# nmndeep/Robust-Segmentation

Hardware: AMD Instinct MI355X
Metric: SEA attack-iterations/sec (UperNet-CNX-T, 512x512) (higher is better)
Workload: dtype f32 (frozen-weight GEMMs on the 16-bit matrix cores by operand splitting: fp16x2 (22 significant bits per operand, 3 MFMA products) forward, fp16x2 (22 significant bits per operand, 3 MFMA products) input gradient; fp32 storage and accumulate)

## Files before the change

devtools/mlp_fused_stamps.py:

```python
#!/usr/bin/env python3
import os
import sys

ROOT = os.path.dirname(os.path.dirname(os.path.abspath(__file__)))
sys.path[:0] = [ROOT, os.path.join(ROOT, "robust-segmentation_amd")]
import torch
from semseg import _native as N

bwd = len(sys.argv) > 1 and sys.argv[1] == "bwd"
C, M = 96, 131072
H = 4 * C
g = torch.Generator(device="cuda").manual_seed(1)
x = torch.randn(M, C, generator=g, device="cuda")
w1 = torch.randn(H, C, generator=g, device="cuda") * 0.05
b1 = torch.randn(H, generator=g, device="cuda") * 0.1
w2 = torch.randn(C, H, generator=g, device="cuda") * 0.03
b2 = torch.randn(C, generator=g, device="cuda") * 0.1
res = torch.randn(M, C, generator=g, device="cuda")
gy = torch.randn(M, C, generator=g, device="cuda") * 1e-3
word = lambda v: torch.tensor([float(v)], dtype=torch.float32, device="cuda").view(torch.int32)
a1, a2 = word(x.abs().max().item() * 1.7), word((x.abs().max() * w1.abs().sum(1) + b1.abs()).max().item())
mul = (w2.abs().sum(0).max() * 1.13).float().reshape(1)
P1, P2 = N.gemm_split_pack(w1, terms=22), N.gemm_split_pack(w2, terms=22)
P2t, P1t = N.gemm_split_pack(w2, trans=True, terms=22), N.gemm_split_pack(w1, trans=True, terms=22)
y = torch.empty(M, C, device="cuda")
WPB = 4
nw = (M + 32 * WPB - 1) // (32 * WPB) * WPB
dbg = torch.zeros(nw, 8, dtype=torch.int64, device="cuda")
p = lambda t: t.data_ptr() if t is not None else None
for _ in range(30):
    N._check(N.lib().sea_mlp_fused_stamps(int(bwd), p(gy), C, p(x), C, p(P1.data), p(b1), p(P2t.data if bwd else P2.data), p(P1t.data),
                                          p(b2), p(res), p(y), M, C, p(a1), p(a2), p(mul), p(dbg), N._stream()), "stamps")
torch.cuda.synchronize()
d = dbg.double().cpu()
names = ["(epilogue, whole kernel: see below)", "interleaved matrix + element-wise work" + (" + first products" if bwd else ""), "wait for the DMA", "barrier"]
tot = d[:, 4].mean().item()
print(f"{'backward' if bwd else 'forward'} C={C} M={M}: {nw} waves, 13 loop iterations, loop total {tot:.0f} ticks per wave (s_memtime = shader cycles)")
for k, n in list(enumerate(names))[1:]:
    print(f"   {n:40s} {d[:, k].mean().item() / 13:8.0f} ticks per iteration   ({100 * d[:, k].mean().item() / tot:4.1f} %)   "
          f"min wave {d[:, k].min().item() / 13:7.0f}  max wave {d[:, k].max().item() / 13:7.0f}")
print(f"   prologue {d[:, 7].mean().item():.0f} ticks per wave (min {d[:, 7].min().item():.0f}, max {d[:, 7].max().item():.0f}); epilogue "
      f"{d[:, 0].mean().item():.0f} (min {d[:, 0].min().item():.0f}, max {d[:, 0].max().item():.0f}); loop {tot:.0f}")
blk = d.view(-1, WPB, 8)
first_round = blk[:256 * 8 // WPB]
print(f"   first 256 blocks: prologue {first_round[:, :, 7].mean().item():.0f}, later blocks: {blk[256 * 8 // WPB:, :, 7].mean().item():.0f}; "
      f"epilogue first {first_round[:, :, 0].mean().item():.0f}, later {blk[256 * 8 // WPB:, :, 0].mean().item():.0f}")
start = d[:, 5]
print(f"   start stamps span {(start.max() - start.min()).item():.0f} ticks over the grid; barrier per wave of a block: "
      + " ".join(f"{blk[:, w, 3].mean().item() / 13:.0f}" for w in range(WPB)))
```

robust-segmentation_amd/csrc/mlp_fused.hip:

```cpp
#include "gemm_split.h"
#include <type_traits>
#include <utility>

namespace sea {

struct MlpArgs {
  const float* x;
  const float* g;
  int64_t ldx, ldg;
  const char* Wa;
  const char* Wu;
  const char* Wb;
  const float* b1;
  const float* b2;
  const float* res;
  int64_t ldres;
  float* y;
  int64_t ldy;
  int M, H, Npad;
  const uint32_t* amax1;
  const uint32_t* amax2;
  unsigned long long* dbg;
  const float* ln_w;
  const float* ln_b;
  float ln_eps;
  const float* amax_mul;
};

__device__ __forceinline__ float erf_small(float x) {
  const float ax = __builtin_fabsf(x);
  const float t = x * x;
  float p = __builtin_fmaf(t, -0x1.268bc2p-11f, 0x1.420828p-8f);
  p = __builtin_fmaf(t, p, -0x1.b5937p-6f);
  p = __builtin_fmaf(t, p, 0x1.ce077cp-4f);
  p = __builtin_fmaf(t, p, -0x1.81266p-2f);
  p = __builtin_fmaf(t, p, 0x1.06eba0p-3f);
  return __builtin_fmaf(ax, p, ax);
}
__device__ __forceinline__ float erf_large_arg(float x) {
  const float ax = __builtin_fabsf(x);
  float q = __builtin_fmaf(ax, 0x1.1d3156p-16f, -0x1.8d129p-12f);
  q = __builtin_fmaf(ax, q, 0x1.f9a6d2p-9f);
  q = __builtin_fmaf(ax, q, -0x1.8c3164p-6f);
  q = __builtin_fmaf(ax, q, 0x1.b4e9c8p-4f);
  q = __builtin_fmaf(ax, q, 0x1.4515fap-1f);
  q = __builtin_fmaf(ax, q, 0x1.078e50p-3f);
  return __builtin_fmaf(ax, q, ax);
}
__device__ __forceinline__ float erf_exp(float q) { return __builtin_expf(-q); }
__device__ __forceinline__ float erf_finish(float x, float small, float ex) {
  return __builtin_copysignf(__builtin_fabsf(x) < 1.0f ? small : 1.0f - ex, x);
}
constexpr float kRsqrt2 = 0.70710678118654752440f;
__device__ __forceinline__ float gelu_finish(float x, float er) { return 0.5f * x * (1.f + er); }
__device__ __forceinline__ float gelu_grad_finish(float x, float er) {
  const float cdf = 0.5f * (1.f + er);
  const float pdf = __expf(-0.5f * x * x) * 0.39894228040143267794f;
  return cdf + x * pdf;
}
__device__ __forceinline__ float erf_nb(float x) { return erf_finish(x, erf_small(x), erf_exp(erf_large_arg(x))); }
__device__ __forceinline__ float gelu_nb(float x) { return gelu_finish(x, erf_nb(x * kRsqrt2)); }
__device__ __forceinline__ float gelu_grad_nb(float x) { return gelu_grad_finish(x, erf_nb(x * kRsqrt2)); }

__global__ __launch_bounds__(256) void gelu_compare_kernel(unsigned long long* out) {
  unsigned long long bad0 = 0, bad1 = 0;
  for (uint64_t i = (uint64_t)blockIdx.x * 256 + threadIdx.x; i < (1ull << 32); i += (uint64_t)gridDim.x * 256) {
    const float x = __uint_as_float((uint32_t)i);
    const float a = gelu_f(x), b = gelu_nb(x), c = gelu_grad_f(x), d = gelu_grad_nb(x);
    bad0 += (__float_as_uint(a) != __float_as_uint(b)) && !(a != a && b != b);
    bad1 += (__float_as_uint(c) != __float_as_uint(d)) && !(c != c && d != d);
  }
  if (bad0) atomicAdd(out, bad0);
  if (bad1) atomicAdd(out + 1, bad1);
}

template <class Fn, int... I>
__device__ __forceinline__ void static_for_impl(Fn&& f, std::integer_sequence<int, I...>) {
  (f(std::integral_constant<int, I>{}), ...);
}
template <int N, class Fn>
__device__ __forceinline__ void static_for(Fn&& f) {
  static_for_impl(f, std::make_integer_sequence<int, N>{});
}


template <int C>
__global__ __launch_bounds__(256) void ln_rows_probe_kernel(const float* x, const float* ln_w, const float* ln_b, float eps, int M,
                                                            float* yn, float* mean, float* rstd) {
  constexpr int KS = C / 16;
  constexpr int LN_KSP = C <= 128 ? 8 : 16;
  const int lane = threadIdx.x & 63, wave = threadIdx.x >> 6;
  const int r = lane & 31, h = lane >> 5;
  int row = (blockIdx.x * 4 + wave) * 32 + r;
  const bool live = row < M;
  row = live ? row : M - 1;
  f32x4 xa[KS][2];
  const float* const xr = x + (int64_t)row * C + 8 * h;
#pragma unroll
  for (int ks = 0; ks < KS; ++ks) {
    xa[ks][0] = *(const f32x4*)(xr + 16 * ks);
    xa[ks][1] = *(const f32x4*)(xr + 16 * ks + 4);
  }
  const float ln_inv_c = 1.f / (float)C;
  auto ln_tree = [&](float (&t)[2][LN_KSP]) __attribute__((always_inline)) -> float {
#pragma unroll
    for (int o = LN_KSP / 2; o > 0; o >>= 1)
#pragma unroll
      for (int i = 0; i < o; ++i) {
        t[0][i] += t[0][i + o];
        t[1][i] += t[1][i + o];
      }
    const float a0 = t[0][0] + __shfl_xor(t[0][0], 32, 64), a1 = t[1][0] + __shfl_xor(t[1][0], 32, 64);
    return a0 + a1;
  };
  float t[2][LN_KSP];
#pragma unroll
  for (int j = 0; j < 2; ++j)
#pragma unroll
    for (int i = 0; i < LN_KSP; ++i) t[j][i] = i < KS ? (xa[i < KS ? i : 0][j][0] + xa[i < KS ? i : 0][j][1]) + (xa[i < KS ? i : 0][j][2] + xa[i < KS ? i : 0][j][3]) : 0.f;
  float mu;
  {
#pragma clang fp contract(off)
    mu = ln_tree(t) * ln_inv_c;
#pragma unroll
    for (int j = 0; j < 2; ++j)
#pragma unroll
      for (int i = 0; i < LN_KSP; ++i) {
        if (i < KS) {
          const float dx = xa[i][j][0] - mu, dy = xa[i][j][1] - mu, dz = xa[i][j][2] - mu, dw = xa[i][j][3] - mu;
          t[j][i] = fmaf(dx, dx, dy * dy) + fmaf(dz, dz, dw * dw);
        } else {
          t[j][i] = 0.f;
        }
      }
  }
  const float rs = rsqrtf(fmaf(ln_tree(t), ln_inv_c, eps));
  if (live) {
#pragma unroll
    for (int ks = 0; ks < KS; ++ks)
#pragma unroll
      for (int j = 0; j < 2; ++j) {
        const f32x4 wv = *(const f32x4*)(ln_w + 16 * ks + 8 * h + 4 * j), bv = *(const f32x4*)(ln_b + 16 * ks + 8 * h + 4 * j);
        f32x4 o;
        {
#pragma clang fp contract(off)
#pragma unroll
          for (int e = 0; e < 4; ++e) o[e] = fmaf((xa[ks][j][e] - mu) * rs, wv[e], bv[e]);
        }
        *(f32x4*)(yn + (int64_t)row * C + 16 * ks + 8 * h + 4 * j) = o;
      }
    if (h == 0) {
      mean[row] = mu;
      rstd[row] = rs;
    }
  }
}

__device__ __forceinline__ f32x16 mfma3(const u32x4 w_hi, const u32x4 w_mid, const u32x4 a_hi, const u32x4 a_mid, f32x16 c) {
  c = __builtin_amdgcn_mfma_f32_32x32x16_f16(__builtin_bit_cast(f16x8, w_hi), __builtin_bit_cast(f16x8, a_mid), c, 0, 0, 0);
  c = __builtin_amdgcn_mfma_f32_32x32x16_f16(__builtin_bit_cast(f16x8, w_mid), __builtin_bit_cast(f16x8, a_hi), c, 0, 0, 0);
  c = __builtin_amdgcn_mfma_f32_32x32x16_f16(__builtin_bit_cast(f16x8, w_hi), __builtin_bit_cast(f16x8, a_hi), c, 0, 0, 0);
  return c;
}

__device__ __forceinline__ void split8(const f32x4 lo, const f32x4 hi4, float sc, u32x4& f_hi, u32x4& f_mid) {
  u32x2 a[2], b[2];
  split4_f16(lo, sc, a);
  split4_f16(hi4, sc, b);
  f_hi = u32x4{a[0][0], a[0][1], b[0][0], b[0][1]};
  f_mid = u32x4{a[1][0], a[1][1], b[1][0], b[1][1]};
}

constexpr int mlp_stage_bytes(int C, bool bwd) { return (bwd ? 3 : 2) * 128 * C; }
constexpr int mlp_cst_bytes(int C, bool bwd) { return (bwd ? 3 : 2) * 4 * C * 4; }
constexpr int mlp_blocks_per_cu(int C, int waves) { return C <= 96 ? 8 / waves : 1; }
constexpr int mlp_lds_bytes(int C, int waves, bool bwd) {
  const int a = 2 * mlp_stage_bytes(C, bwd) + mlp_cst_bytes(C, bwd);
  const int b = waves * 32 * (C + 4) * 4;
  return a > b ? a : b;
}

template <int C, int WAVES, bool BWD, bool PIPE, bool STAMP = false>
__global__ __launch_bounds__(WAVES * 64, (C <= 96 ? 8 : 4) / 4) void mlp_fused_kernel(const MlpArgs p) {
  constexpr int T = WAVES * 64;
  constexpr int KS = C / 16;
  constexpr int NT = C / 32;
  constexpr int ARR = 128 * C;
  constexpr int NARR = BWD ? 3 : 2;
  constexpr int STAGE = NARR * ARR;
  constexpr int PIECES = STAGE / 16;
  constexpr int PER = (PIECES + T - 1) / T;
  static_assert(PIECES % 64 == 0, "whole waves of 16-byte pieces");
  extern __shared__ __attribute__((aligned(16))) char smem[];

  const uint64_t t_entry = STAMP ? __builtin_amdgcn_s_memtime() : 0;
  const int tid = threadIdx.x, lane = tid & 63, wave = tid >> 6;
  const int wave_u = __builtin_amdgcn_readfirstlane(wave);
  const int r = lane & 31, h = lane >> 5;
  const int M = p.M, H = p.H;
  const int NTILE = H / 32;
  const int m0 = ((int)blockIdx.x * WAVES + wave) * 32;
  int row = m0 + r;
  const bool live = row < M;
  row = live ? row : M - 1;

  const uint32_t lane_off = (uint32_t)((lane >> 2) * 64 + (((lane & 3) ^ ((lane >> 4) & 3)) * 16));
  auto dma = [&](char* st, int ja, int jb) __attribute__((always_inline)) {
    ja = ja < NTILE ? ja : NTILE - 1;
    jb = jb < NTILE ? jb : NTILE - 1;
#pragma unroll
    for (int i = 0; i < PER; ++i) {
      const int pcw = wave_u * 64 + T * i;
      if (PIECES % T != 0 && pcw >= PIECES) continue;
      const int arr = pcw / (8 * C), qw = pcw - arr * (8 * C);
      const char* src;
      if (arr < NARR - 1)
        src = (arr == 0 ? p.Wa : p.Wu) + ((int64_t)(qw >> 7) * H + 32 * ja) * 64 + (qw & 127) * 16;
      else {
        const int t = qw / (4 * C);
        src = p.Wb + ((int64_t)(2 * jb + t) * p.Npad) * 64 + (qw - t * (4 * C)) * 16;
      }
      __builtin_amdgcn_global_load_lds((const __attribute__((address_space(1))) void*)(src + lane_off),
                                       (__attribute__((address_space(3))) void*)(st + pcw * 16), 16, 0, 0);
    }
  };
  char* const st0 = smem;
  char* const st1 = smem + STAGE;
  float* const cst = (float*)(smem + 2 * STAGE);
  {
    const float* const wa_g = (const float*)(p.Wa + (int64_t)(C / 32) * 2 * H * 64);
    const float* const wu_g = BWD ? (const float*)(p.Wu + (int64_t)(C / 32) * 2 * H * 64) : nullptr;
    for (int i = tid; i < H; i += T) {
      cst[i] = wa_g[i];
      cst[H + i] = p.b1[i];
      if constexpr (BWD) cst[2 * H + i] = wu_g[i];
    }
  }
  dma(st1, 0, 0);
  dma(st0, 1, 0);

  constexpr int LDP = (C + 4) * 4;
  constexpr int NF4 = 32 * C / 4 / 64;
  auto load_rows = [&](const float* base, int64_t ld, f32x4 (&out)[KS][2]) __attribute__((always_inline)) {
    const float* const xr = base + (int64_t)row * ld + 8 * h;
#pragma unroll
    for (int ks = 0; ks < KS; ++ks) {
      out[ks][0] = *(const f32x4*)(xr + 16 * ks);
      out[ks][1] = *(const f32x4*)(xr + 16 * ks + 4);
    }
  };
  float sc1, inv1;
  pow2_scale(*p.amax1, sc1, inv1);
  u32x4 xf[KS][2];
  constexpr int LN_KSP = C <= 128 ? 8 : 16;
  const float ln_inv_c = 1.f / (float)C;
  auto ln_tree = [&](float (&t)[2][LN_KSP]) __attribute__((always_inline)) -> float {
#pragma unroll
    for (int o = LN_KSP / 2; o > 0; o >>= 1)
#pragma unroll
      for (int i = 0; i < o; ++i) {
        t[0][i] += t[0][i + o];
        t[1][i] += t[1][i + o];
      }
    const float a0 = t[0][0] + __shfl_xor(t[0][0], 32, 64), a1 = t[1][0] + __shfl_xor(t[1][0], 32, 64);
    return a0 + a1;
  };
  float ln_mu = 0.f, ln_rs = 1.f;
  {
    f32x4 xa[KS][2];
    load_rows(p.x, p.ldx, xa);
    if (p.ln_w != nullptr) {
      float t[2][LN_KSP];
#pragma unroll
      for (int j = 0; j < 2; ++j)
#pragma unroll
        for (int i = 0; i < LN_KSP; ++i) t[j][i] = i < KS ? (xa[i < KS ? i : 0][j][0] + xa[i < KS ? i : 0][j][1]) + (xa[i < KS ? i : 0][j][2] + xa[i < KS ? i : 0][j][3]) : 0.f;
      {
#pragma clang fp contract(off)
        ln_mu = ln_tree(t) * ln_inv_c;
#pragma unroll
        for (int j = 0; j < 2; ++j)
#pragma unroll
          for (int i = 0; i < LN_KSP; ++i) {
            if (i < KS) {
              const float dx = xa[i][j][0] - ln_mu, dy = xa[i][j][1] - ln_mu, dz = xa[i][j][2] - ln_mu, dw = xa[i][j][3] - ln_mu;
              t[j][i] = fmaf(dx, dx, dy * dy) + fmaf(dz, dz, dw * dw);
            } else {
              t[j][i] = 0.f;
            }
          }
      }
      ln_rs = rsqrtf(fmaf(ln_tree(t), ln_inv_c, p.ln_eps));
#pragma unroll
      for (int ks = 0; ks < KS; ++ks)
#pragma unroll
        for (int j = 0; j < 2; ++j) {
          const f32x4 wv = *(const f32x4*)(p.ln_w + 16 * ks + 8 * h + 4 * j), bv = *(const f32x4*)(p.ln_b + 16 * ks + 8 * h + 4 * j);
          {
#pragma clang fp contract(off)
#pragma unroll
            for (int e = 0; e < 4; ++e) xa[ks][j][e] = fmaf((xa[ks][j][e] - ln_mu) * ln_rs, wv[e], bv[e]);
          }
        }
    }
#pragma unroll
    for (int ks = 0; ks < KS; ++ks) split8(xa[ks][0], xa[ks][1], sc1, xf[ks][0], xf[ks][1]);
  }
  float sc2 = 1.f, inv2 = 1.f;
  float invg = 1.f;
  u32x4 gf[BWD ? KS : 1][2];
  if constexpr (BWD) {
    f32x4 ga[KS][2];
    load_rows(p.g, p.ldg, ga);
    uint32_t mx = 0;
#pragma unroll
    for (int ks = 0; ks < KS; ++ks) {
#pragma unroll
      for (int e = 0; e < 4; ++e) {
        const uint32_t b0 = __float_as_uint(ga[ks][0][e]) & 0x7fffffffu, b1 = __float_as_uint(ga[ks][1][e]) & 0x7fffffffu;
        mx = b0 > mx ? b0 : mx;
        mx = b1 > mx ? b1 : mx;
      }
    }
    const uint32_t other = (uint32_t)__shfl_xor((int)mx, 32, 64);
    mx = other > mx ? other : mx;
    float scg;
    pow2_scale(mx, scg, invg);
    const float mul = *p.amax_mul;
    uint32_t word = mx;
    if (mul != 1.f) word = __float_as_uint(__uint_as_float(word) * mul) & 0x7fffffffu;
    pow2_scale(word, sc2, inv2);
#pragma unroll
    for (int ks = 0; ks < KS; ++ks) split8(ga[ks][0], ga[ks][1], scg, gf[ks][0], gf[ks][1]);
  } else {
    pow2_scale(*p.amax2, sc2, inv2);
  }

  asm volatile("s_waitcnt vmcnt(0)" ::: "memory");
  __syncthreads();

  const uint32_t rd = (uint32_t)(r * 64 + swz<false>(r, h));
  auto first = [&](const char* st, f32x16& Tt, f32x16& Ut) __attribute__((always_inline)) {
#pragma unroll
    for (int e = 0; e < 16; ++e) Tt[e] = 0.f;
    if constexpr (BWD) {
#pragma unroll
      for (int e = 0; e < 16; ++e) Ut[e] = 0.f;
    }
#pragma unroll
    for (int ks = 0; ks < KS; ++ks) {
      const uint32_t o = (uint32_t)((ks >> 1) * 4096) + (rd ^ (uint32_t)(32 * (ks & 1)));
      const u32x4 w0 = *(const u32x4*)(st + o), w1 = *(const u32x4*)(st + o + 2048);
      Tt = mfma3(w0, w1, xf[ks][0], xf[ks][1], Tt);
      if constexpr (BWD) {
        const u32x4 u0 = *(const u32x4*)(st + ARR + o), u1 = *(const u32x4*)(st + ARR + o + 2048);
        Ut = mfma3(u0, u1, gf[ks][0], gf[ks][1], Ut);
      }
    }
  };

  f32x16 acc[NT];
#pragma unroll
  for (int n = 0; n < NT; ++n)
#pragma unroll
    for (int e = 0; e < 16; ++e) acc[n][e] = 0.f;

  f32x16 Tc, Uc, Tn, Un;
  first(st1, Tc, Uc);
  __syncthreads();

  const float* const wi_a = cst;
  const float* const b1_l = cst + H;
  const float* const wi_u = cst + 2 * H;
  constexpr int SECOND = (NARR - 1) * ARR;

  u32x4 hp[2][2] = {};
  uint64_t tick[4] = {0, 0, 0, 0};
  const uint64_t t_begin = STAMP ? __builtin_amdgcn_s_memtime() : 0;
#define SEA_PIN() __builtin_amdgcn_sched_barrier(0)
  auto body = [&](auto FF, auto SS, auto EE, int j) __attribute__((always_inline)) {
    constexpr bool F = decltype(FF)::value, S = decltype(SS)::value, E = decltype(EE)::value;
    char* const cur = (j & 1) ? st1 : st0;
    char* const nxt = (j & 1) ? st0 : st1;
    uint64_t c0 = 0, c2 = 0, c3 = 0, c4 = 0;
    if constexpr (STAMP) {
      c0 = __builtin_amdgcn_s_memtime();
      SEA_PIN();
    }
    constexpr bool LAG = PIPE;
    if (j + 1 < NTILE + (LAG ? 1 : 0)) dma(nxt, j + 2, LAG ? j : j + 1);
    constexpr int NTF = (F && PIPE) ? (BWD ? 2 : 1) * KS : 0;
    constexpr int NTS = (S && LAG) ? 2 * NT : 0;
    constexpr int NTR = NTF + NTS, NM = 3 * NTR;
    u32x4 wf[2][2];
    auto rd_frags = [&](auto TR) __attribute__((always_inline)) {
      constexpr int tr = decltype(TR)::value;
      if constexpr (tr < NTF) {
        constexpr int ks = BWD ? tr >> 1 : tr;
        const uint32_t o = (uint32_t)(((BWD && (tr & 1)) ? ARR : 0) + (ks >> 1) * 4096) + (rd ^ (uint32_t)(32 * (ks & 1)));
        wf[tr & 1][0] = *(const u32x4*)(cur + o);
        wf[tr & 1][1] = *(const u32x4*)(cur + o + 2048);
      } else {
        constexpr int t2 = tr - NTF, ss = t2 / NT, n = t2 - ss * NT;
        const uint32_t o = (uint32_t)(SECOND + n * 2048) + (rd ^ (uint32_t)(32 * ss));
        wf[tr & 1][0] = *(const u32x4*)(cur + o);
        wf[tr & 1][1] = *(const u32x4*)(cur + o + C * 64);
      }
    };
    auto mfma_m = [&](auto MC) __attribute__((always_inline)) {
      constexpr int m = decltype(MC)::value, tr = m / 3, pr = m - 3 * tr;
      if constexpr (pr == 0 && tr + 1 < NTR) rd_frags(std::integral_constant<int, tr + 1>{});
      const f16x8 w = __builtin_bit_cast(f16x8, wf[tr & 1][pr == 1 ? 1 : 0]);
      constexpr int at = pr == 0 ? 1 : 0;
      if constexpr (tr < NTF) {
        constexpr int ks = BWD ? tr >> 1 : tr;
        if constexpr (BWD && (tr & 1)) {
          if constexpr (tr == 1 && pr == 0) {
#pragma unroll
            for (int e = 0; e < 16; ++e) Un[e] = 0.f;
          }
          Un = __builtin_amdgcn_mfma_f32_32x32x16_f16(w, __builtin_bit_cast(f16x8, gf[BWD ? ks : 0][at]), Un, 0, 0, 0);
        } else {
          if constexpr (tr == 0 && pr == 0) {
#pragma unroll
            for (int e = 0; e < 16; ++e) Tn[e] = 0.f;
          }
          Tn = __builtin_amdgcn_mfma_f32_32x32x16_f16(w, __builtin_bit_cast(f16x8, xf[ks][at]), Tn, 0, 0, 0);
        }
      } else {
        constexpr int t2 = tr - NTF, ss = t2 / NT, n = t2 - ss * NT;
        acc[n] = __builtin_amdgcn_mfma_f32_32x32x16_f16(w, __builtin_bit_cast(f16x8, hp[ss][at]), acc[n], 0, 0, 0);
      }
    };
    if constexpr (NTR > 0) rd_frags(std::integral_constant<int, 0>{});
    u32x4 hf[2][2];
    if constexpr (E) {
      constexpr int EPS = 4;
      constexpr int SPQ = 2 + 4 * (4 / EPS);
      constexpr int NSTEP = 4 * SPQ + 1;
      float ev[16], ek[16], ep[16], eq[16];
      uint32_t hq[4][2], mq[4][2];
      f32x4 wa, bb, wu;
      auto cst_rd = [&](int q) __attribute__((always_inline)) {
        const int hid = 32 * j + 8 * q + 4 * h;
        wa = *(const f32x4*)(wi_a + hid);
        bb = *(const f32x4*)(b1_l + hid);
        if constexpr (BWD) wu = *(const f32x4*)(wi_u + hid);
      };
      cst_rd(0);
      static_for<NSTEP>([&](auto IC) __attribute__((always_inline)) {
        constexpr int i = decltype(IC)::value;
        constexpr int m0 = i * NM / NSTEP, m1 = (i + 1) * NM / NSTEP;
        static_for<m1 - m0>([&](auto U) __attribute__((always_inline)) { mfma_m(std::integral_constant<int, m0 + decltype(U)::value>{}); });
        constexpr int q = i / SPQ, k = i - SPQ * q;
        if constexpr (i == NSTEP - 1) {
#pragma unroll
          for (int s2 = 0; s2 < 2; ++s2) {
            const auto a0 = __builtin_amdgcn_permlane32_swap(hq[2 * s2][0], hq[2 * s2 + 1][0], false, false);
            const auto a1 = __builtin_amdgcn_permlane32_swap(hq[2 * s2][1], hq[2 * s2 + 1][1], false, false);
            const auto b0 = __builtin_amdgcn_permlane32_swap(mq[2 * s2][0], mq[2 * s2 + 1][0], false, false);
            const auto b1 = __builtin_amdgcn_permlane32_swap(mq[2 * s2][1], mq[2 * s2 + 1][1], false, false);
            hf[s2][0] = u32x4{a0[0], a1[0], a0[1], a1[1]};
            hf[s2][1] = u32x4{b0[0], b1[0], b0[1], b1[1]};
          }
        } else if constexpr (k == 0) {
#pragma unroll
          for (int e = 0; e < 4; ++e) {
            const float t = Tc[4 * q + e] * (inv1 * wa[e]) + bb[e];
            ev[4 * q + e] = t;
            ek[4 * q + e] = t * kRsqrt2;
          }
        } else if constexpr (k == SPQ - 1) {
          u32x2 s2[2];
          split4_f16(f32x4{ev[4 * q], ev[4 * q + 1], ev[4 * q + 2], ev[4 * q + 3]}, sc2, s2);
          hq[q][0] = s2[0][0];
          hq[q][1] = s2[0][1];
          mq[q][0] = s2[1][0];
          mq[q][1] = s2[1][1];
          if constexpr (q + 1 < 4) cst_rd(q + 1);
        } else {
          constexpr int pr = (k - 1) >> 2, st = (k - 1) & 3;
#pragma unroll
          for (int d = 0; d < EPS; ++d) {
            const int e = 4 * q + EPS * pr + d;
            if constexpr (st == 0) ep[e] = erf_small(ek[e]);
            if constexpr (st == 1) eq[e] = erf_large_arg(ek[e]);
            if constexpr (st == 2) eq[e] = erf_exp(eq[e]);
            if constexpr (st == 3) {
              const float er = erf_finish(ek[e], ep[e], eq[e]);
              if constexpr (BWD) {
                float u = Uc[e] * (invg * wu[e & 3]) + 0.f;
                u *= gelu_grad_finish(ev[e], er);
                ev[e] = u;
              } else {
                ev[e] = gelu_finish(ev[e], er);
              }
            }
          }
        }
        SEA_PIN();
      });
    } else {
      static_for<NM>([&](auto MC) __attribute__((always_inline)) { mfma_m(MC); });
    }
    if constexpr (S && !LAG) {
#pragma unroll
      for (int ss = 0; ss < 2; ++ss)
#pragma unroll
        for (int n = 0; n < NT; ++n) {
          const uint32_t o = (uint32_t)(SECOND + n * 2048) + (rd ^ (uint32_t)(32 * ss));
          const u32x4 w0 = *(const u32x4*)(cur + o), w1 = *(const u32x4*)(cur + o + C * 64);
          acc[n] = mfma3(w0, w1, hf[ss][0], hf[ss][1], acc[n]);
        }
    }
    if constexpr (F && !PIPE) first(cur, Tc, Uc);
    if constexpr (E && LAG) {
#pragma unroll
      for (int s2 = 0; s2 < 2; ++s2) {
        hp[s2][0] = hf[s2][0];
        hp[s2][1] = hf[s2][1];
      }
    }
    if constexpr (STAMP) {
      SEA_PIN();
      c2 = __builtin_amdgcn_s_memtime();
      SEA_PIN();
    }
    asm volatile("s_waitcnt vmcnt(0)" ::: "memory");
    if constexpr (STAMP) {
      c3 = __builtin_amdgcn_s_memtime();
      SEA_PIN();
    }
    __syncthreads();
    if constexpr (STAMP) {
      c4 = __builtin_amdgcn_s_memtime();
      SEA_PIN();
      tick[0] += 0;
      tick[1] += c2 - c0;
      tick[2] += c3 - c2;
      tick[3] += c4 - c3;
    }
    if constexpr (F && PIPE) {
      Tc = Tn;
      if constexpr (BWD) Uc = Un;
    }
  };
#undef SEA_PIN
  using Y = std::true_type;
  using No = std::false_type;
  if constexpr (PIPE) {
    body(Y{}, No{}, Y{}, 0);
    for (int j = 1; j + 1 < NTILE; ++j) body(Y{}, Y{}, Y{}, j);
    body(No{}, Y{}, Y{}, NTILE - 1);
    body(No{}, Y{}, No{}, NTILE);
  } else {
    for (int j = 0; j + 1 < NTILE; ++j) body(Y{}, Y{}, Y{}, j);
    body(No{}, Y{}, Y{}, NTILE - 1);
  }
  const uint64_t t_loop_end = STAMP ? __builtin_amdgcn_s_memtime() : 0;

  const float* const wi_b = (const float*)(p.Wb + (int64_t)(H / 32) * 2 * p.Npad * 64);
  {
    char* const ep = smem + wave_u * (32 * LDP);
#pragma unroll
    for (int n = 0; n < NT; ++n)
#pragma unroll
      for (int q = 0; q < 4; ++q) {
        const int col = 32 * n + 8 * q + 4 * h;
        const f32x4 wb = *(const f32x4*)(wi_b + col);
        f32x4 bb = {0.f, 0.f, 0.f, 0.f};
        if (!BWD && p.b2) bb = *(const f32x4*)(p.b2 + col);
        f32x4 v;
#pragma unroll
        for (int e = 0; e < 4; ++e) v[e] = acc[n][4 * q + e] * (inv2 * wb[e]) + bb[e];
        if constexpr (BWD) {
          if (p.ln_w != nullptr) {
#pragma unroll
            for (int e = 0; e < 4; ++e) acc[n][4 * q + e] = v[e];
            continue;
          }
        }
        *(f32x4*)(ep + r * LDP + col * 4) = v;
      }
    if constexpr (BWD) {
      if (p.ln_w != nullptr) {
        constexpr int NTP = C <= 128 ? 4 : 8;
        const float* const xr = p.x + (int64_t)row * p.ldx;
        float t1[NTP][4], t2[NTP][4];
        f32x4 gw[NT][4], xh[NT][4];
#pragma unroll
        for (int n = 0; n < NTP; ++n)
#pragma unroll
          for (int q = 0; q < 4; ++q) {
            if (n < NT) {
              const int col = 32 * n + 8 * q + 4 * h;
              const f32x4 wv = *(const f32x4*)(p.ln_w + col), xv = *(const f32x4*)(xr + col);
              const int nn = n < NT ? n : 0;
              {
#pragma clang fp contract(off)
#pragma unroll
                for (int e = 0; e < 4; ++e) {
                  gw[nn][q][e] = acc[nn][4 * q + e] * wv[e];
                  xh[nn][q][e] = (xv[e] - ln_mu) * ln_rs;
                }
                t1[n][q] = (gw[nn][q][0] + gw[nn][q][1]) + (gw[nn][q][2] + gw[nn][q][3]);
                t2[n][q] = (gw[nn][q][0] * xh[nn][q][0] + gw[nn][q][1] * xh[nn][q][1]) + (gw[nn][q][2] * xh[nn][q][2] + gw[nn][q][3] * xh[nn][q][3]);
              }
            } else {
              t1[n][q] = 0.f;
              t2[n][q] = 0.f;
            }
          }
#pragma unroll
        for (int o = NTP / 2; o > 0; o >>= 1)
#pragma unroll
          for (int i = 0; i < o; ++i)
#pragma unroll
            for (int q = 0; q < 4; ++q) {
              t1[i][q] += t1[i + o][q];
              t2[i][q] += t2[i + o][q];
            }
        float s1 = (t1[0][0] + t1[0][2]) + (t1[0][1] + t1[0][3]), s2 = (t2[0][0] + t2[0][2]) + (t2[0][1] + t2[0][3]);
        s1 += __shfl_xor(s1, 32, 64);
        s2 += __shfl_xor(s2, 32, 64);
#pragma unroll
        for (int n = 0; n < NT; ++n)
#pragma unroll
          for (int q = 0; q < 4; ++q) {
            f32x4 o4;
            {
#pragma clang fp contract(off)
              const float m1 = s1 * ln_inv_c, m2 = s2 * ln_inv_c;
#pragma unroll
              for (int e = 0; e < 4; ++e) o4[e] = ln_rs * fmaf(-xh[n][q][e], m2, gw[n][q][e] - m1);
            }
            *(f32x4*)(ep + r * LDP + (32 * n + 8 * q + 4 * h) * 4) = o4;
          }
      }
    }
    const bool has_res = !BWD && p.res != nullptr;
#pragma unroll
    for (int it = 0; it < NF4; ++it) {
      const int f = lane + 64 * it, rw = f / (C / 4), c4 = f - rw * (C / 4);
      f32x4 v = *(const f32x4*)(ep + rw * LDP + c4 * 16);
      if (m0 + rw < M) {
        if (has_res) v += *(const f32x4*)(p.res + (int64_t)(m0 + rw) * p.ldres + 4 * c4);
        *(f32x4*)(p.y + (int64_t)(m0 + rw) * p.ldy + 4 * c4) = v;
      }
    }
  }
  if constexpr (STAMP) {
    asm volatile("s_waitcnt vmcnt(0)" ::: "memory");
    if (lane == 0 && p.dbg) {
      unsigned long long* d = p.dbg + ((int64_t)blockIdx.x * WAVES + wave) * 8;
      for (int k = 1; k < 4; ++k) d[k] = tick[k];
      d[0] = __builtin_amdgcn_s_memtime() - t_loop_end;
      d[4] = t_loop_end - t_begin;
      d[5] = t_begin;
      d[6] = __builtin_amdgcn_s_memrealtime();
      d[7] = t_begin - t_entry;
    }
  }
}

template <int C, int WAVES, bool BWD, bool PIPE, bool STAMP = false>
static int mlp_launch(const MlpArgs& p, hipStream_t st) {
  constexpr int lds = mlp_lds_bytes(C, WAVES, BWD);
  static_assert(lds * mlp_blocks_per_cu(C, WAVES) <= 160 * 1024, "LDS of a compute unit");
  auto k = mlp_fused_kernel<C, WAVES, BWD, PIPE, STAMP>;
  if (lds > 48 * 1024) {
    static bool attr_set_dev[64] = {};
    int dev = 0;
    (void)hipGetDevice(&dev);
    if (!attr_set_dev[dev & 63]) {
      (void)hipFuncSetAttribute((const void*)k, hipFuncAttributeMaxDynamicSharedMemorySize, lds);
      attr_set_dev[dev & 63] = true;
    }
  }
  const int rows_per_block = WAVES * 32;
  hipLaunchKernelGGL(k, dim3((p.M + rows_per_block - 1) / rows_per_block), dim3(WAVES * 64), (size_t)lds, st, p);
  return (int)hipGetLastError();
}

}

using namespace sea;

extern "C" int sea_probe_gelu_mismatches(unsigned long long* out, void* stream) {
  SEA_CHECK_ARG(out != nullptr);
  hipLaunchKernelGGL(gelu_compare_kernel, dim3(256 * 16), dim3(256), 0, (hipStream_t)stream, out);
  SEA_RETURN_LAST();
}

extern "C" int sea_probe_ln_rows(const float* x, const float* ln_w, const float* ln_b, float eps, int M, int C, float* yn, float* mean,
                                 float* rstd, void* stream) {
  SEA_CHECK_ARG(x && ln_w && ln_b && yn && mean && rstd && M > 0 && (C == 96 || C == 192));
  const dim3 grid((M + 127) / 128), block(256);
  if (C == 96)
    hipLaunchKernelGGL(ln_rows_probe_kernel<96>, grid, block, 0, (hipStream_t)stream, x, ln_w, ln_b, eps, M, yn, mean, rstd);
  else
    hipLaunchKernelGGL(ln_rows_probe_kernel<192>, grid, block, 0, (hipStream_t)stream, x, ln_w, ln_b, eps, M, yn, mean, rstd);
  SEA_RETURN_LAST();
}

extern "C" int sea_mlp_fused_supported(int C, int H) { return (H == 4 * C && (C == 96 || C == 192)) ? 1 : 0; }

static bool mlp_common_ok(const MlpArgs& p, int C) {
  return p.x && p.Wa && p.Wb && p.b1 && p.y && p.amax1 && p.M > 0 && sea_mlp_fused_supported(C, p.H) && (p.ldx % 4) == 0 &&
         (p.ldy % 4) == 0 && p.ldx >= C && p.ldy >= C &&
         ((((uintptr_t)p.x) | ((uintptr_t)p.y) | ((uintptr_t)p.Wa) | ((uintptr_t)p.Wb) | ((uintptr_t)p.b1)) & 15) == 0;
}

static int mlp_fwd_impl(const float* x, int64_t ldx, const void* W1p, const float* b1, const void* W2p, const float* b2,
                        const float* res, int64_t ldres, float* y, int64_t ldy, int M, int C, int H, const uint32_t* amax_x,
                        const uint32_t* amax_h, const float* ln_w, const float* ln_b, float ln_eps, void* stream) {
  MlpArgs p = {};
  p.ln_w = ln_w; p.ln_b = ln_b; p.ln_eps = ln_eps;
  SEA_CHECK_ARG((ln_w == nullptr) == (ln_b == nullptr) && ((((uintptr_t)ln_w) | ((uintptr_t)ln_b)) & 15) == 0);
  p.x = x; p.ldx = ldx; p.Wa = (const char*)W1p; p.Wb = (const char*)W2p; p.b1 = b1; p.b2 = b2; p.res = res; p.ldres = ldres;
  p.y = y; p.ldy = ldy; p.M = M; p.H = H; p.Npad = (C + GS_BN - 1) / GS_BN * GS_BN; p.amax1 = amax_x; p.amax2 = amax_h;
  SEA_CHECK_ARG(mlp_common_ok(p, C) && amax_h != nullptr);
  SEA_CHECK_ARG((((uintptr_t)b2) & 15) == 0 && (!res || ((ldres % 4) == 0 && ldres >= C && (((uintptr_t)res) & 15) == 0)));
  const hipStream_t st = (hipStream_t)stream;
  if (C == 96) return mlp_launch<96, 4, false, true>(p, st);
  return mlp_launch<192, 4, false, true>(p, st);
}

extern "C" int sea_mlp_fused_fwd(const float* x, int64_t ldx, const void* W1p, const float* b1, const void* W2p, const float* b2,
                                 const float* res, int64_t ldres, float* y, int64_t ldy, int M, int C, int H,
                                 const uint32_t* amax_x, const uint32_t* amax_h, void* stream) {
  return mlp_fwd_impl(x, ldx, W1p, b1, W2p, b2, res, ldres, y, ldy, M, C, H, amax_x, amax_h, nullptr, nullptr, 0.f, stream);
}
extern "C" int sea_ln_mlp_fused_fwd(const float* x, int64_t ldx, const float* ln_w, const float* ln_b, float ln_eps, const void* W1p,
                                    const float* b1, const void* W2p, const float* b2, const float* res, int64_t ldres, float* y,
                                    int64_t ldy, int M, int C, int H, const uint32_t* amax_x, const uint32_t* amax_h, void* stream) {
  SEA_CHECK_ARG(ln_w && ln_b);
  return mlp_fwd_impl(x, ldx, W1p, b1, W2p, b2, res, ldres, y, ldy, M, C, H, amax_x, amax_h, ln_w, ln_b, ln_eps, stream);
}

static int mlp_bwd_impl(const float* g, int64_t ldg, const float* x, int64_t ldx, const void* W1p, const float* b1,
                        const void* W2tp, const void* W1tp, float* dx, int64_t lddx, int M, int C, int H, const uint32_t* amax_x,
                        const float* amax_mul_dev, const float* ln_w, const float* ln_b, float ln_eps, void* stream) {
  MlpArgs p = {};
  p.ln_w = ln_w; p.ln_b = ln_b; p.ln_eps = ln_eps;
  SEA_CHECK_ARG((ln_w == nullptr) == (ln_b == nullptr) && ((((uintptr_t)ln_w) | ((uintptr_t)ln_b)) & 15) == 0);
  p.x = x; p.ldx = ldx; p.g = g; p.ldg = ldg; p.Wa = (const char*)W1p; p.Wu = (const char*)W2tp; p.Wb = (const char*)W1tp;
  p.b1 = b1; p.y = dx; p.ldy = lddx; p.M = M; p.H = H; p.Npad = (C + GS_BN - 1) / GS_BN * GS_BN; p.amax1 = amax_x;
  p.amax_mul = amax_mul_dev;
  SEA_CHECK_ARG(mlp_common_ok(p, C) && g && W2tp && amax_mul_dev && (ldg % 4) == 0 && ldg >= C &&
                ((((uintptr_t)g) | ((uintptr_t)W2tp)) & 15) == 0);
  const hipStream_t st = (hipStream_t)stream;
  if (C == 96) return mlp_launch<96, 4, true, false>(p, st);
  return mlp_launch<192, 4, true, true>(p, st);
}

extern "C" int sea_mlp_fused_bwd(const float* g, int64_t ldg, const float* x, int64_t ldx, const void* W1p, const float* b1,
                                 const void* W2tp, const void* W1tp, float* dx, int64_t lddx, int M, int C, int H,
                                 const uint32_t* amax_x, const float* amax_mul_dev, void* stream) {
  return mlp_bwd_impl(g, ldg, x, ldx, W1p, b1, W2tp, W1tp, dx, lddx, M, C, H, amax_x, amax_mul_dev, nullptr, nullptr, 0.f, stream);
}
extern "C" int sea_ln_mlp_fused_bwd(const float* g, int64_t ldg, const float* x, int64_t ldx, const float* ln_w, const float* ln_b,
                                    float ln_eps, const void* W1p, const float* b1, const void* W2tp, const void* W1tp, float* dx,
                                    int64_t lddx, int M, int C, int H, const uint32_t* amax_x, const float* amax_mul_dev,
                                    void* stream) {
  SEA_CHECK_ARG(ln_w && ln_b);
  return mlp_bwd_impl(g, ldg, x, ldx, W1p, b1, W2tp, W1tp, dx, lddx, M, C, H, amax_x, amax_mul_dev, ln_w, ln_b, ln_eps, stream);
}

extern "C" int sea_mlp_fused_stamps(int bwd, const float* g, int64_t ldg, const float* x, int64_t ldx, const void* W1p, const float* b1,
                                    const void* W2p, const void* W1tp, const float* b2, const float* res, float* y, int M, int C,
                                    const uint32_t* amax_x, const uint32_t* amax_h, const float* amax_mul_dev,
                                    unsigned long long* dbg, void* stream) {
  SEA_CHECK_ARG(C == 96 && dbg && x && y);
  MlpArgs p = {};
  p.x = x; p.ldx = ldx; p.g = g; p.ldg = ldg; p.Wa = (const char*)W1p; p.b1 = b1; p.y = y; p.ldy = C; p.M = M; p.H = 4 * C;
  p.Npad = (C + GS_BN - 1) / GS_BN * GS_BN; p.amax1 = amax_x; p.amax2 = amax_h; p.amax_mul = amax_mul_dev; p.dbg = dbg;
  if (bwd) {
    p.Wu = (const char*)W2p; p.Wb = (const char*)W1tp;
    return mlp_launch<96, 4, true, false, true>(p, (hipStream_t)stream);
  }
  p.Wb = (const char*)W2p; p.b2 = b2; p.res = res; p.ldres = C;
  return mlp_launch<96, 4, false, true, true>(p, (hipStream_t)stream);
}
```

Measured before the change: 571.3.

## Split C=192 fused MLP forward across wave pairs with LDS exchange

For the C=192 forward MLP, each 32-row group is now handled by two waves (8 waves per block). One wave runs the first GEMM and half the GELU/split epilogue, the other does the remaining epilogue quarters and the second GEMM. They exchange hidden fragments and T values through a double-buffered LDS slot. This aims to raise occupancy and overlap matrix and element-wise work at the C=192 stage, at the cost of extra LDS, barriers and a role imbalance between the two waves.

```diff
diff --git a/devtools/mlp_fused_stamps.py b/devtools/mlp_fused_stamps.py
--- a/devtools/mlp_fused_stamps.py
+++ b/devtools/mlp_fused_stamps.py
@@ -8,7 +8,8 @@
 from semseg import _native as N
 
 bwd = len(sys.argv) > 1 and sys.argv[1] == "bwd"
-C, M = 96, 131072
+C = int(sys.argv[2]) if len(sys.argv) > 2 else 96
+M = 131072 if C == 96 else 32768
 H = 4 * C
 g = torch.Generator(device="cuda").manual_seed(1)
 x = torch.randn(M, C, generator=g, device="cuda")
@@ -24,8 +25,10 @@
 P1, P2 = N.gemm_split_pack(w1, terms=22), N.gemm_split_pack(w2, terms=22)
 P2t, P1t = N.gemm_split_pack(w2, trans=True, terms=22), N.gemm_split_pack(w1, trans=True, terms=22)
 y = torch.empty(M, C, device="cuda")
-WPB = 4
-nw = (M + 32 * WPB - 1) // (32 * WPB) * WPB
+WPB = int(sys.argv[3]) if len(sys.argv) > 3 else (8 if C == 192 and not bwd else 4)
+RPB = 128
+nw = (M + RPB - 1) // RPB * WPB
+NIT = H // 32 + 1
 dbg = torch.zeros(nw, 8, dtype=torch.int64, device="cuda")
 p = lambda t: t.data_ptr() if t is not None else None
 for _ in range(30):
@@ -35,10 +38,10 @@
 d = dbg.double().cpu()
 names = ["(epilogue, whole kernel: see below)", "interleaved matrix + element-wise work" + (" + first products" if bwd else ""), "wait for the DMA", "barrier"]
 tot = d[:, 4].mean().item()
-print(f"{'backward' if bwd else 'forward'} C={C} M={M}: {nw} waves, 13 loop iterations, loop total {tot:.0f} ticks per wave (s_memtime = shader cycles)")
+print(f"{'backward' if bwd else 'forward'} C={C} M={M}: {nw} waves, {NIT} loop iterations, loop total {tot:.0f} ticks per wave (s_memtime = shader cycles)")
 for k, n in list(enumerate(names))[1:]:
-    print(f"   {n:40s} {d[:, k].mean().item() / 13:8.0f} ticks per iteration   ({100 * d[:, k].mean().item() / tot:4.1f} %)   "
-          f"min wave {d[:, k].min().item() / 13:7.0f}  max wave {d[:, k].max().item() / 13:7.0f}")
+    print(f"   {n:40s} {d[:, k].mean().item() / NIT:8.0f} ticks per iteration   ({100 * d[:, k].mean().item() / tot:4.1f} %)   "
+          f"min wave {d[:, k].min().item() / NIT:7.0f}  max wave {d[:, k].max().item() / NIT:7.0f}")
 print(f"   prologue {d[:, 7].mean().item():.0f} ticks per wave (min {d[:, 7].min().item():.0f}, max {d[:, 7].max().item():.0f}); epilogue "
       f"{d[:, 0].mean().item():.0f} (min {d[:, 0].min().item():.0f}, max {d[:, 0].max().item():.0f}); loop {tot:.0f}")
 blk = d.view(-1, WPB, 8)
@@ -47,4 +50,7 @@
       f"epilogue first {first_round[:, :, 0].mean().item():.0f}, later {blk[256 * 8 // WPB:, :, 0].mean().item():.0f}")
 start = d[:, 5]
 print(f"   start stamps span {(start.max() - start.min()).item():.0f} ticks over the grid; barrier per wave of a block: "
-      + " ".join(f"{blk[:, w, 3].mean().item() / 13:.0f}" for w in range(WPB)))
+      + " ".join(f"{blk[:, w, 3].mean().item() / NIT:.0f}" for w in range(WPB)))
+print("   per wave of a block, work ticks per iteration: " + " ".join(f"{blk[:, w, 1].mean().item() / NIT:.0f}" for w in range(WPB))
+      + "; prologue: " + " ".join(f"{blk[:, w, 7].mean().item():.0f}" for w in range(WPB))
+      + "; epilogue: " + " ".join(f"{blk[:, w, 0].mean().item():.0f}" for w in range(WPB)))
diff --git a/robust-segmentation_amd/csrc/mlp_fused.hip b/robust-segmentation_amd/csrc/mlp_fused.hip
--- a/robust-segmentation_amd/csrc/mlp_fused.hip
+++ b/robust-segmentation_amd/csrc/mlp_fused.hip
@@ -173,16 +173,22 @@
 
 constexpr int mlp_stage_bytes(int C, bool bwd) { return (bwd ? 3 : 2) * 128 * C; }
 constexpr int mlp_cst_bytes(int C, bool bwd) { return (bwd ? 3 : 2) * 4 * C * 4; }
+constexpr bool mlp_paired(int C, bool bwd) { return C == 192 && !bwd; }
+constexpr int mlp_groups(int C, int waves, bool bwd) { return mlp_paired(C, bwd) ? waves / 2 : waves; }
+constexpr int mlp_xchg_bytes(int C, int waves, bool bwd) { return mlp_paired(C, bwd) ? (waves / 2) * 2 * 4096 : 0; }
 constexpr int mlp_blocks_per_cu(int C, int waves) { return C <= 96 ? 8 / waves : 1; }
 constexpr int mlp_lds_bytes(int C, int waves, bool bwd) {
-  const int a = 2 * mlp_stage_bytes(C, bwd) + mlp_cst_bytes(C, bwd);
-  const int b = waves * 32 * (C + 4) * 4;
+  const int a = 2 * mlp_stage_bytes(C, bwd) + mlp_cst_bytes(C, bwd) + mlp_xchg_bytes(C, waves, bwd);
+  const int b = mlp_groups(C, waves, bwd) * 32 * (C + 4) * 4;
   return a > b ? a : b;
 }
 
 template <int C, int WAVES, bool BWD, bool PIPE, bool STAMP = false>
-__global__ __launch_bounds__(WAVES * 64, (C <= 96 ? 8 : 4) / 4) void mlp_fused_kernel(const MlpArgs p) {
+__global__ __launch_bounds__(WAVES * 64, (C <= 96 || mlp_paired(C, BWD)) ? 2 : 1) void mlp_fused_kernel(const MlpArgs p) {
   constexpr int T = WAVES * 64;
+  constexpr bool PAIR = mlp_paired(C, BWD);
+  constexpr int GROUPS = mlp_groups(C, WAVES, BWD);
+  static_assert(!PAIR || (PIPE && WAVES == 8), "the paired form is the pipelined loop at two waves per SIMD");
   constexpr int KS = C / 16;
   constexpr int NT = C / 32;
   constexpr int ARR = 128 * C;
@@ -199,7 +205,8 @@
   const int r = lane & 31, h = lane >> 5;
   const int M = p.M, H = p.H;
   const int NTILE = H / 32;
-  const int m0 = ((int)blockIdx.x * WAVES + wave) * 32;
+  const int grp = PAIR ? wave_u % GROUPS : wave_u, role = PAIR ? wave_u / GROUPS : 0;
+  const int m0 = ((int)blockIdx.x * GROUPS + grp) * 32;
   int row = m0 + r;
   const bool live = row < M;
   row = live ? row : M - 1;
@@ -227,6 +234,7 @@
   char* const st0 = smem;
   char* const st1 = smem + STAGE;
   float* const cst = (float*)(smem + 2 * STAGE);
+  char* const xch = smem + 2 * STAGE + mlp_cst_bytes(C, BWD) + grp * 8192 + lane * 16;
   {
     const float* const wa_g = (const float*)(p.Wa + (int64_t)(C / 32) * 2 * H * 64);
     const float* const wu_g = BWD ? (const float*)(p.Wu + (int64_t)(C / 32) * 2 * H * 64) : nullptr;
@@ -266,7 +274,7 @@
     return a0 + a1;
   };
   float ln_mu = 0.f, ln_rs = 1.f;
-  {
+  auto load_x = [&]() __attribute__((always_inline)) {
     f32x4 xa[KS][2];
     load_rows(p.x, p.ldx, xa);
     if (p.ln_w != nullptr) {
@@ -305,7 +313,8 @@
     }
 #pragma unroll
     for (int ks = 0; ks < KS; ++ks) split8(xa[ks][0], xa[ks][1], sc1, xf[ks][0], xf[ks][1]);
-  }
+  };
+  if constexpr (!PAIR) load_x();
   float sc2 = 1.f, inv2 = 1.f;
   float invg = 1.f;
   u32x4 gf[BWD ? KS : 1][2];
@@ -336,8 +345,11 @@
     pow2_scale(*p.amax2, sc2, inv2);
   }
 
-  asm volatile("s_waitcnt vmcnt(0)" ::: "memory");
-  __syncthreads();
+  auto landed = [&]() __attribute__((always_inline)) {
+    asm volatile("s_waitcnt vmcnt(0)" ::: "memory");
+    __syncthreads();
+  };
+  if constexpr (!PAIR) landed();
 
   const uint32_t rd = (uint32_t)(r * 64 + swz<false>(r, h));
   auto first = [&](const char* st, f32x16& Tt, f32x16& Ut) __attribute__((always_inline)) {
@@ -366,8 +378,10 @@
     for (int e = 0; e < 16; ++e) acc[n][e] = 0.f;
 
   f32x16 Tc, Uc, Tn, Un;
-  first(st1, Tc, Uc);
-  __syncthreads();
+  if constexpr (!PAIR) {
+    first(st1, Tc, Uc);
+    __syncthreads();
+  }
 
   const float* const wi_a = cst;
   const float* const b1_l = cst + H;
@@ -376,10 +390,11 @@
 
   u32x4 hp[2][2] = {};
   uint64_t tick[4] = {0, 0, 0, 0};
-  const uint64_t t_begin = STAMP ? __builtin_amdgcn_s_memtime() : 0;
+  uint64_t t_begin = (STAMP && !PAIR) ? __builtin_amdgcn_s_memtime() : 0;
 #define SEA_PIN() __builtin_amdgcn_sched_barrier(0)
-  auto body = [&](auto FF, auto SS, auto EE, int j) __attribute__((always_inline)) {
+  auto body = [&](auto FF, auto SS, auto EE, auto RRC, int j) __attribute__((always_inline)) {
     constexpr bool F = decltype(FF)::value, S = decltype(SS)::value, E = decltype(EE)::value;
+    constexpr int RR = decltype(RRC)::value;
     char* const cur = (j & 1) ? st1 : st0;
     char* const nxt = (j & 1) ? st0 : st1;
     uint64_t c0 = 0, c2 = 0, c3 = 0, c4 = 0;
@@ -434,10 +449,23 @@
     };
     if constexpr (NTR > 0) rd_frags(std::integral_constant<int, 0>{});
     u32x4 hf[2][2];
+    f32x4 te[2];
+    if constexpr (RR == 2) {
+      const char* const sl = xch + ((j + 1) & 1) * 4096;
+      if constexpr (S) {
+        hp[0][0] = *(const u32x4*)(sl);
+        hp[0][1] = *(const u32x4*)(sl + 1024);
+      }
+      if constexpr (E) {
+        te[0] = *(const f32x4*)(sl + 2048);
+        te[1] = *(const f32x4*)(sl + 3072);
+      }
+    }
     if constexpr (E) {
       constexpr int EPS = 4;
       constexpr int SPQ = 2 + 4 * (4 / EPS);
-      constexpr int NSTEP = 4 * SPQ + 1;
+      constexpr int NQ = RR ? 2 : 4, QB = RR == 2 ? 2 : 0;
+      constexpr int NSTEP = NQ * SPQ + 1;
       float ev[16], ek[16], ep[16], eq[16];
       uint32_t hq[4][2], mq[4][2];
       f32x4 wa, bb, wu;
@@ -447,7 +475,7 @@
         bb = *(const f32x4*)(b1_l + hid);
         if constexpr (BWD) wu = *(const f32x4*)(wi_u + hid);
       };
-      cst_rd(0);
+      cst_rd(QB);
       static_for<NSTEP>([&](auto IC) __attribute__((always_inline)) {
         constexpr int i = decltype(IC)::value;
         constexpr int m0 = i * NM / NSTEP, m1 = (i + 1) * NM / NSTEP;
@@ -455,18 +483,21 @@
         constexpr int q = i / SPQ, k = i - SPQ * q;
         if constexpr (i == NSTEP - 1) {
 #pragma unroll
-          for (int s2 = 0; s2 < 2; ++s2) {
+          for (int s2 = 0; s2 < NQ / 2; ++s2) {
             const auto a0 = __builtin_amdgcn_permlane32_swap(hq[2 * s2][0], hq[2 * s2 + 1][0], false, false);
             const auto a1 = __builtin_amdgcn_permlane32_swap(hq[2 * s2][1], hq[2 * s2 + 1][1], false, false);
             const auto b0 = __builtin_amdgcn_permlane32_swap(mq[2 * s2][0], mq[2 * s2 + 1][0], false, false);
             const auto b1 = __builtin_amdgcn_permlane32_swap(mq[2 * s2][1], mq[2 * s2 + 1][1], false, false);
-            hf[s2][0] = u32x4{a0[0], a1[0], a0[1], a1[1]};
-            hf[s2][1] = u32x4{b0[0], b1[0], b0[1], b1[1]};
+            hf[QB / 2 + s2][0] = u32x4{a0[0], a1[0], a0[1], a1[1]};
+            hf[QB / 2 + s2][1] = u32x4{b0[0], b1[0], b0[1], b1[1]};
           }
         } else if constexpr (k == 0) {
 #pragma unroll
           for (int e = 0; e < 4; ++e) {
-            const float t = Tc[4 * q + e] * (inv1 * wa[e]) + bb[e];
+            float tq;
+            if constexpr (RR == 2) tq = te[q][e];
+            else tq = Tc[4 * q + e];
+            const float t = tq * (inv1 * wa[e]) + bb[e];
             ev[4 * q + e] = t;
             ek[4 * q + e] = t * kRsqrt2;
           }
@@ -477,7 +508,7 @@
           hq[q][1] = s2[0][1];
           mq[q][0] = s2[1][0];
           mq[q][1] = s2[1][1];
-          if constexpr (q + 1 < 4) cst_rd(q + 1);
+          if constexpr (q + 1 < NQ) cst_rd(QB + q + 1);
         } else {
           constexpr int pr = (k - 1) >> 2, st = (k - 1) & 3;
 #pragma unroll
@@ -514,11 +545,22 @@
         }
     }
     if constexpr (F && !PIPE) first(cur, Tc, Uc);
-    if constexpr (E && LAG) {
-#pragma unroll
-      for (int s2 = 0; s2 < 2; ++s2) {
+    if constexpr (E && LAG && RR != 1) {
+#pragma unroll
+      for (int s2 = RR ? 1 : 0; s2 < 2; ++s2) {
         hp[s2][0] = hf[s2][0];
         hp[s2][1] = hf[s2][1];
+      }
+    }
+    if constexpr (RR == 1) {
+      char* const sl = xch + (j & 1) * 4096;
+      if constexpr (E) {
+        *(u32x4*)(sl) = hf[0][0];
+        *(u32x4*)(sl + 1024) = hf[0][1];
+      }
+      if constexpr (F) {
+        *(f32x4*)(sl + 2048) = f32x4{Tn[8], Tn[9], Tn[10], Tn[11]};
+        *(f32x4*)(sl + 3072) = f32x4{Tn[12], Tn[13], Tn[14], Tn[15]};
       }
     }
     if constexpr (STAMP) {
@@ -546,22 +588,9 @@
     }
   };
 #undef SEA_PIN
-  using Y = std::true_type;
-  using No = std::false_type;
-  if constexpr (PIPE) {
-    body(Y{}, No{}, Y{}, 0);
-    for (int j = 1; j + 1 < NTILE; ++j) body(Y{}, Y{}, Y{}, j);
-    body(No{}, Y{}, Y{}, NTILE - 1);
-    body(No{}, Y{}, No{}, NTILE);
-  } else {
-    for (int j = 0; j + 1 < NTILE; ++j) body(Y{}, Y{}, Y{}, j);
-    body(No{}, Y{}, Y{}, NTILE - 1);
-  }
-  const uint64_t t_loop_end = STAMP ? __builtin_amdgcn_s_memtime() : 0;
-
   const float* const wi_b = (const float*)(p.Wb + (int64_t)(H / 32) * 2 * p.Npad * 64);
-  {
-    char* const ep = smem + wave_u * (32 * LDP);
+  char* const ep = smem + grp * (32 * LDP);
+  auto to_patch = [&]() __attribute__((always_inline)) {
 #pragma unroll
     for (int n = 0; n < NT; ++n)
 #pragma unroll
@@ -582,6 +611,46 @@
         }
         *(f32x4*)(ep + r * LDP + col * 4) = v;
       }
+  };
+  uint64_t t_loop_end = 0;
+  using Y = std::true_type;
+  using No = std::false_type;
+  using R0 = std::integral_constant<int, 0>;
+  if constexpr (PAIR) {
+    if (role == 0) {
+      load_x();
+      landed();
+      first(st1, Tc, Uc);
+      *(f32x4*)(xch + 4096 + 2048) = f32x4{Tc[8], Tc[9], Tc[10], Tc[11]};
+      *(f32x4*)(xch + 4096 + 3072) = f32x4{Tc[12], Tc[13], Tc[14], Tc[15]};
+      __syncthreads();
+      if constexpr (STAMP) t_begin = __builtin_amdgcn_s_memtime();
+      for (int j = 0; j + 1 < NTILE; ++j) body(Y{}, No{}, Y{}, std::integral_constant<int, 1>{}, j);
+      body(No{}, No{}, Y{}, std::integral_constant<int, 1>{}, NTILE - 1);
+      body(No{}, No{}, No{}, std::integral_constant<int, 1>{}, NTILE);
+    } else {
+      landed();
+      __syncthreads();
+      if constexpr (STAMP) t_begin = __builtin_amdgcn_s_memtime();
+      body(No{}, No{}, Y{}, std::integral_constant<int, 2>{}, 0);
+      for (int j = 1; j < NTILE; ++j) body(No{}, Y{}, Y{}, std::integral_constant<int, 2>{}, j);
+      body(No{}, Y{}, No{}, std::integral_constant<int, 2>{}, NTILE);
+      if constexpr (STAMP) t_loop_end = __builtin_amdgcn_s_memtime();
+      to_patch();
+    }
+  } else if constexpr (PIPE) {
+    body(Y{}, No{}, Y{}, R0{}, 0);
+    for (int j = 1; j + 1 < NTILE; ++j) body(Y{}, Y{}, Y{}, R0{}, j);
+    body(No{}, Y{}, Y{}, R0{}, NTILE - 1);
+    body(No{}, Y{}, No{}, R0{}, NTILE);
+  } else {
+    for (int j = 0; j + 1 < NTILE; ++j) body(Y{}, Y{}, Y{}, R0{}, j);
+    body(No{}, Y{}, Y{}, R0{}, NTILE - 1);
+  }
+  if (STAMP && !(PAIR && role == 1)) t_loop_end = __builtin_amdgcn_s_memtime();
+
+  {
+    if constexpr (!PAIR) to_patch();
     if constexpr (BWD) {
       if (p.ln_w != nullptr) {
         constexpr int NTP = C <= 128 ? 4 : 8;
@@ -639,8 +708,11 @@
       }
     }
     const bool has_res = !BWD && p.res != nullptr;
-#pragma unroll
-    for (int it = 0; it < NF4; ++it) {
+    if constexpr (PAIR) __syncthreads();
+    constexpr int NIT = PAIR ? NF4 / 2 : NF4;
+#pragma unroll
+    for (int i = 0; i < NIT; ++i) {
+      const int it = PAIR ? role * NIT + i : i;
       const int f = lane + 64 * it, rw = f / (C / 4), c4 = f - rw * (C / 4);
       f32x4 v = *(const f32x4*)(ep + rw * LDP + c4 * 16);
       if (m0 + rw < M) {
@@ -677,7 +749,7 @@
       attr_set_dev[dev & 63] = true;
     }
   }
-  const int rows_per_block = WAVES * 32;
+  const int rows_per_block = mlp_groups(C, WAVES, BWD) * 32;
   hipLaunchKernelGGL(k, dim3((p.M + rows_per_block - 1) / rows_per_block), dim3(WAVES * 64), (size_t)lds, st, p);
   return (int)hipGetLastError();
 }
@@ -723,7 +795,7 @@
   SEA_CHECK_ARG((((uintptr_t)b2) & 15) == 0 && (!res || ((ldres % 4) == 0 && ldres >= C && (((uintptr_t)res) & 15) == 0)));
   const hipStream_t st = (hipStream_t)stream;
   if (C == 96) return mlp_launch<96, 4, false, true>(p, st);
-  return mlp_launch<192, 4, false, true>(p, st);
+  return mlp_launch<192, 8, false, true>(p, st);
 }
 
 extern "C" int sea_mlp_fused_fwd(const float* x, int64_t ldx, const void* W1p, const float* b1, const void* W2p, const float* b2,
@@ -771,14 +843,16 @@
                                     const void* W2p, const void* W1tp, const float* b2, const float* res, float* y, int M, int C,
                                     const uint32_t* amax_x, const uint32_t* amax_h, const float* amax_mul_dev,
                                     unsigned long long* dbg, void* stream) {
-  SEA_CHECK_ARG(C == 96 && dbg && x && y);
+  SEA_CHECK_ARG((C == 96 || C == 192) && dbg && x && y);
   MlpArgs p = {};
   p.x = x; p.ldx = ldx; p.g = g; p.ldg = ldg; p.Wa = (const char*)W1p; p.b1 = b1; p.y = y; p.ldy = C; p.M = M; p.H = 4 * C;
   p.Npad = (C + GS_BN - 1) / GS_BN * GS_BN; p.amax1 = amax_x; p.amax2 = amax_h; p.amax_mul = amax_mul_dev; p.dbg = dbg;
   if (bwd) {
     p.Wu = (const char*)W2p; p.Wb = (const char*)W1tp;
+    if (C == 192) return mlp_launch<192, 4, true, true, true>(p, (hipStream_t)stream);
     return mlp_launch<96, 4, true, false, true>(p, (hipStream_t)stream);
   }
   p.Wb = (const char*)W2p; p.b2 = b2; p.res = res; p.ldres = C;
+  if (C == 192) return mlp_launch<192, 8, false, true, true>(p, (hipStream_t)stream);
   return mlp_launch<96, 4, false, true, true>(p, (hipStream_t)stream);
 }
```

After: 574.2, median of 6. Within noise of the previous version (+0.5%).
